# nipponjo/tts-arabic-pytorch

Hardware: AMD Instinct MI355X
Metric: audio samples/sec (FastPitch+HiFi-GAN, synthetic 64-phoneme inputs) (higher is better)
Workload: dtype f32

## Files before the change

tts-arabic-pytorch_amd/csrc/api.hip:

```cpp
#include <cerrno>
#include <cstdio>
#include <cstdlib>
#include <cstring>
#include <algorithm>
#include <atomic>
#include <mutex>
#include <string>
#include <vector>

#include "kernels.hpp"

namespace ttsamd {

static thread_local std::string g_err;

void set_error(const char* fmt, ...) {
    char buf[1024];
    va_list ap;
    va_start(ap, fmt);
    vsnprintf(buf, sizeof(buf), fmt, ap);
    va_end(ap);
    g_err = buf;
}

// ... 436 lines not shown
    TTS_REQUIRE(mode >= 0 && mode <= 2 && (mode != 2 || div != 0.f), "conv1d: bad mode / div");
    TTS_REQUIRE(relu_out == 0 || mode == 0, "conv1d: relu_out with an accumulate mode (mode %d) is not defined", mode);
    hipStream_t s = (hipStream_t)stream;
    const int cp = cout_padded(cout);
    const int64_t n = (int64_t)cin * k * cp;
    hipLaunchKernelGGL(pack_conv_weight_kernel, dim3((unsigned)((n + 255) / 256)), dim3(256), 0, s, w, cout, cin, k,
                       cp, packed);
    TTS_CHECK_HIP(hipGetLastError());
    ConvParams p;
    std::memset(&p, 0, sizeof(p));
    p.x = x; p.x_bs = (int64_t)cin * lin; p.x_cs = lin;
    p.w = packed; p.bias = bias;
    p.precision = default_precision();
    if (p.precision != 0) {
        unsigned short* planes = reinterpret_cast<unsigned short*>(packed + n);
        hipLaunchKernelGGL(split_bf16_kernel, dim3((unsigned)((n + 255) / 256)), dim3(256), 0, s, packed, n, planes);
        TTS_CHECK_HIP(hipGetLastError());
        p.w_bf16 = planes;
    }
    if ((k == 3 || k == 7 || k == 11) && p.precision == 0 && cin % 8 == 0) {
        float* wino = packed + 2 * n;
        const int64_t nw = (int64_t)cin * wino2_groups(k) * cp;
        hipLaunchKernelGGL(pack_wino2_weight_kernel, dim3((unsigned)((nw + 255) / 256)), dim3(256), 0, s, w, cout, cin, k, cp, wino);
        TTS_CHECK_HIP(hipGetLastError());
        p.w_wino = wino;
        float* wino4 = wino + nw;
        const int64_t nw4 = (int64_t)cin * wino4_groups(k) * cp;
        hipLaunchKernelGGL(pack_wino4_weight_kernel, dim3((unsigned)((nw4 + 255) / 256)), dim3(256), 0, s, w, cout, cin, k, cp, wino4);
        TTS_CHECK_HIP(hipGetLastError());
        p.w_wino4 = wino4;
    }
    p.y = y; p.y_bs = (int64_t)cout * lin; p.y_cs = lin; p.y_ts = 1;
    p.lens_in = lens; p.lens_out = lens; p.len_in_mul = 1; p.len_out_mul = 1;
    p.Lin = lin; p.Nout = lin; p.Cin = cin; p.Cout = cout; p.CoutP = cp; p.K = k;
    p.dil = dilation; p.pad = (k * dilation - dilation) / 2;
    p.res = res; p.r_bs = (int64_t)cout * lin; p.r_cs = lin;
    p.n_phase = 1; p.in_slope = in_slope; p.relu_out = relu_out; p.mode = mode; p.div = div; p.batch = batch;
    prof_begin(s, 2.0 * cout * cin * k);
    const int32_t rc = launch_conv(p, s);
    prof_end(s);
    return rc;
}

int32_t ttsamd_conv1d(const float* x, const float* w, const float* bias, const int64_t* lens, int32_t batch,
                      int32_t cin, int32_t cout, int32_t k, int32_t dilation, int32_t lin, float in_slope,
                      int32_t relu_out, float* y, float* packed, void* stream) {
    return ttsamd_conv1d_ex(x, w, bias, nullptr, lens, batch, cin, cout, k, dilation, lin, in_slope, relu_out, 0, 1.f, y, packed, stream);
}

int64_t ttsamd_resblock_pair_packed_floats(int32_t channels, int32_t k, int32_t variant) {
    if (channels < 1 || k < 1) return 0;
    const int64_t n = 2 * (int64_t)channels * k * channels;
    const int nwino = (variant == 4 ? 1 : (variant == 5 ? 2 : 0));
    return n + ((k == 3 || k == 7 || k == 11) ? nwino * (int64_t)channels * wino2_groups(k) * channels : 0);
}

int32_t ttsamd_resblock_pair(const float* x, float* y, const float* w1, const float* b1, const float* w2, const float* b2,
                             int32_t channels, int32_t k, int32_t dil, const int64_t* lens, int32_t len_mul, int32_t L,
                             int32_t batch, int32_t mode, float div, float slope, int32_t variant, float* packed, int64_t packed_floats,
                             void* stream) {
    TTS_REQUIRE(x && y && w1 && b1 && w2 && b2 && packed && channels % 32 == 0 && k >= 1 && batch >= 1 && L >= 1 && len_mul >= 1 &&
                mode >= 0 && mode <= 2, "resblock_pair: bad argument");
    TTS_REQUIRE(packed_floats >= ttsamd_resblock_pair_packed_floats(channels, k, variant),
                "resblock_pair: `packed` holds %lld floats, variant %d at C = %d, k = %d needs %lld (ttsamd_resblock_pair_packed_floats)",
                (long long)packed_floats, variant, channels, k, (long long)ttsamd_resblock_pair_packed_floats(channels, k, variant));
    hipStream_t s = (hipStream_t)stream;
    const int64_t n = (int64_t)channels * k * channels;
    for (int i = 0; i < 2; ++i) {
        hipLaunchKernelGGL(pack_conv_weight_kernel, dim3((unsigned)((n + 255) / 256)), dim3(256), 0, s, i == 0 ? w1 : w2, channels,
                           channels, k, channels, packed + i * n);
        TTS_CHECK_HIP(hipGetLastError());
    }
    const double fl = 2.0 * (2.0 * channels * channels * k);
    int32_t rc;
    prof_begin(s, fl);
    if (variant == 1) {
        rc = launch_fused_pair(channels, x, y, packed, b1, packed + n, b2, k, dil, lens, len_mul, L, batch, mode, div, slope, s);
    } else if (variant >= 2 && variant <= 5) {
        const float *w2w = nullptr, *w1w = nullptr;
        if (variant >= 4) {
            TTS_REQUIRE((k == 3 || k == 7 || k == 11) && (channels <= 64 || (variant == 5 && channels == 128)),
                        "resblock_pair: variants 4 / 5 are built for C = 32 / 64 (5: and 128), k = 3 / 7 / 11");
            const int64_t nw = (int64_t)channels * wino2_groups(k) * channels;
            for (int i = 0; i < (variant == 5 ? 2 : 1); ++i) {
                float* wino = packed + 2 * n + i * nw;
                hipLaunchKernelGGL(pack_wino2_weight_kernel, dim3((unsigned)((nw + 255) / 256)), dim3(256), 0, s, i == 0 ? w2 : w1, channels,
                                   channels, k, channels, wino);
                TTS_CHECK_HIP(hipGetLastError());
                (i == 0 ? w2w : w1w) = wino;
            }
        }
        rc = launch_fused_pair2(channels, x, y, packed, b1, packed + n, b2, k, dil, lens, len_mul, L, batch, mode, div, slope,
                                variant == 3 ? 1 : 2, s, w2w, w1w);
    } else if (variant == -1) {
        rc = 0;
    } else {
        set_error("resblock_pair: variant %d (1: first generation, 2 / 3: second generation with 256- / 128-column blocks, 4 / 5: 256 columns + Winograd phase B / both phases)", variant);
        rc = TTSAMD_EINVAL;
    }
    prof_end(s);
    return rc;
}

int32_t ttsamd_set_precision(int32_t precision) {
    TTS_REQUIRE(precision >= 0 && precision <= 2, "set_precision: 0 = fp32 MFMA, 1 = bf16 MFMA, 2 = split-bf16 MFMA");
    g_precision = precision;
    return 0;
}
int32_t ttsamd_get_precision(void) { return g_precision; }

int32_t ttsamd_profile_enable(int32_t on) {
    std::lock_guard<std::mutex> lk(g_prof.mu);
    g_prof.on = on != 0;
    g_prof.used = 0;
    g_prof.launches = 0;
    g_prof.flops_per_frame = 0.0;
    return 0;
}

int32_t ttsamd_profile_read(double* out3) {
    TTS_REQUIRE(out3, "profile_read: null argument");
    std::lock_guard<std::mutex> lk(g_prof.mu);
    std::vector<std::pair<float, float>> iv;
    for (size_t i = 0; i + 1 < g_prof.used; i += 2) {
        TTS_CHECK_HIP(hipEventSynchronize(g_prof.ev[i + 1]));
        float t0 = 0.f, t1 = 0.f;
        if (i > 0) TTS_CHECK_HIP(hipEventElapsedTime(&t0, g_prof.ev[0], g_prof.ev[i]));
        TTS_CHECK_HIP(hipEventElapsedTime(&t1, g_prof.ev[0], g_prof.ev[i + 1]));
        iv.emplace_back(t0, std::max(t0, t1));
    }
    std::sort(iv.begin(), iv.end());
    double ms = 0.0;
    float lo = 0.f, hi = -1.f;
    for (const auto& v : iv) {
        if (hi < lo || v.first > hi) {
            if (hi >= lo) ms += hi - lo;
            lo = v.first;
            hi = v.second;
        } else {
            hi = std::max(hi, v.second);
        }
    }
    if (hi >= lo) ms += hi - lo;
    out3[0] = ms;
    out3[1] = (double)g_prof.launches;
    out3[2] = (double)(g_prof.used / 2);
    return 0;
}

}
// ... 1 lines not shown
```

tts-arabic-pytorch_amd/csrc/common.hpp:

```cpp
#pragma once
#include <hip/hip_runtime.h>
#include <stdint.h>
#include <atomic>
#include <cstdarg>
#include <cstdio>
#include <cstdlib>
#include <string>

#include "../../include/ttsamd.h"

namespace ttsamd {

void set_error(const char* fmt, ...);

#define TTS_CHECK_HIP(expr)                                                         \
    do {                                                                            \
        hipError_t e_ = (expr);                                                     \
        if (e_ != hipSuccess) {                                                     \
            ttsamd::set_error("%s failed: %s (%s:%d)", #expr, hipGetErrorString(e_), \
                              __FILE__, __LINE__);                                  \
            return TTSAMD_EHIP;                                                     \
        }                                                                           \
    } while (0)

#define TTS_REQUIRE(cond, ...)              \
    do {                                    \
        if (!(cond)) {                      \
            ttsamd::set_error(__VA_ARGS__); \
            return TTSAMD_EINVAL;           \
        }                                   \
    } while (0)

#define TTS_TRY(expr)               \
    do {                            \
        int32_t rc_ = (expr);       \
        if (rc_ != 0) return rc_;   \
    } while (0)

inline int64_t align_up(int64_t x, int64_t a) { return (x + a - 1) / a * a; }

inline const char* exp_env(const char* name) {
#ifdef TTS_EXPERIMENT
    return std::getenv(name);
#else
    (void)name;
    return nullptr;
#endif
}

inline hipError_t lds_opt_in(const void* fn, int bytes, std::atomic<uint64_t>& done) {
    int dev = 0;
    hipError_t e = hipGetDevice(&dev);
    if (e != hipSuccess) return e;
    if (dev >= 0 && dev < 64 && ((done.load(std::memory_order_acquire) >> dev) & 1)) return hipSuccess;
    e = hipFuncSetAttribute(fn, hipFuncAttributeMaxDynamicSharedMemorySize, bytes);
    if (e == hipSuccess && dev >= 0 && dev < 64) done.fetch_or(1ull << dev, std::memory_order_release);
    return e;
}

#define TTS_OPTIONS(X)                                                                                     \
    X(HIFIGAN_STREAMS, 0, 0, 1)    \
    X(WINO, 0, 0, 1)                                              \
    X(WINO2, 0, 0, 31)             \
    X(WINO4, 0, 0, 31)             \
    X(FUSED_PAIR, 0, 0, 1)                   \
    X(FUSED2, 0, 0, 1)                                           \
    X(FUSED2_MASK, 1, 0, 0x1ff)               \
    X(FUSED2_MASK_N1, 1, 0, 0x1ff)          \
    X(FUSED2_WB, 0, 0, 2)                     \
    X(CONVT, 0, 0, 1)                              \
    X(BFO, 0, 0, 1)                \
    X(BFO_CHAIN, 0, 0, 1)                           \
    X(BFO_CHAIN7, 0, 0, 1)                                 \
    X(BFO_FF, 0, 0, 1)                              \
    X(BFO_SPLITK, 0, 0, 1)                                              \
    X(BFO_SMALL_TILES, 0, 0, 1)            \
    X(BF16_ATTN, 0, 0, 1)                                         \
    X(BF16_PACKED_T, 0, 0, 1)                   \
    X(ATT_RA, 0, 1, 4)                             \
    X(ATT_SPLIT, 0, 0, 1)                      \
    X(XCD_W, 0, 0, 1)                            \
    X(XCD_WMAX_KB, 0, 0, 1 << 20)     \
    X(DEEP_SPLITK, 0, 0, 1)        \
    X(TACO_PERSISTENT, 0, 0, 2)    \
    X(TACO_SEG, 0, 8, 1 << 20)
enum Opt : int {
#define TTS_OPT_ENUM(name, kind, lo, hi) OPT_##name,
    TTS_OPTIONS(TTS_OPT_ENUM)
#undef TTS_OPT_ENUM
    OPT_COUNT
};
const char* opt_str(Opt o);

struct Arena {
    char* base;
    int64_t size;
    int64_t off = 0;
    bool ok = true;
    Arena(void* p, int64_t n) : base((char*)p), size(n) {}
    template <typename T>
    T* take(int64_t count) {
        int64_t bytes = align_up(count * (int64_t)sizeof(T), 256);
        if (base != nullptr && off + bytes > size) ok = false;
        T* r = base ? (T*)(base + off) : nullptr;
        off += bytes;
        return r;
    }
};

struct ConvParams {
    const float* x;
    int64_t x_bs;
    int32_t x_cs;
    const float* w;
    const void* w_bf16;
    const float* w_wino;
    const float* w_wino4;
    int32_t precision;
    const float* bias;
    float* y;
    int64_t y_bs;
    int32_t y_cs, y_ts;
    const float* res;
    int64_t r_bs;
    int32_t r_cs;
    const int64_t* lens_in;
    const int64_t* lens_out;
    int32_t len_in_mul, len_out_mul;
    int32_t Lin, Nout;
    int32_t Cin, Cout, CoutP, K;
    int32_t dil, pad;
    int32_t n_phase;
    int32_t phase_p;
    float in_slope;
    const float* scale;
    int32_t relu_out;
    int32_t mode;
    float div;
    int32_t batch;
    float* splitk_ws;
    int64_t splitk_floats;
    int32_t ksplit;
    int32_t y_packed;
    float pack_slope;
    int32_t x_packed;
    int32_t xcd_w;
    int32_t tile_major;
    int32_t compact;
    unsigned long long* timing;
};
constexpr int64_t kSplitKFloats = 4 << 20;
constexpr int64_t kSplitKFloatsFp = 8 << 20;

void conv_log(const char* kind, int K, int cin, int cout, int nout, int batch, int has_res, int mode, int len_mul, int ragged,
              int n_phase);
bool tile_major_order(const ConvParams& p, unsigned n_tiles);
bool compact_order(const void* lens, int batch);
int32_t launch_conv(const ConvParams& p, hipStream_t stream);
bool convt_supported(const ConvParams& p);
int32_t launch_convt(const ConvParams& p, hipStream_t stream);
bool fused_pair_supported(int32_t channels, int32_t k, int32_t dil, int32_t L, const float* x, const float* y);
int32_t launch_fused_pair(int32_t channels, const float* x, float* y, const float* w1, const float* b1, const float* w2,
                          const float* b2, int32_t k, int32_t dil, const int64_t* lens, int32_t len_mul, int32_t L, int32_t batch,
                          int32_t mode, float div, float slope, hipStream_t stream);
bool fused_pair2_supported(int32_t channels, int32_t k, int32_t dil, int32_t L, const float* x, const float* y, int32_t ntw);
int32_t launch_fused_pair2(int32_t channels, const float* x, float* y, const float* w1, const float* b1, const float* w2,
                           const float* b2, int32_t k, int32_t dil, const int64_t* lens, int32_t len_mul, int32_t L, int32_t batch,
                           int32_t mode, float div, float slope, int32_t ntw, hipStream_t stream, const float* w2_wino = nullptr,
                           const float* w1_wino = nullptr);
int wino_route(const ConvParams& p);
int32_t launch_wino(const ConvParams& p, hipStream_t stream);
void pack_wino_weight(const float* w, int cout, int cin, float* out);
int wino2_groups(int k);
int wino2_block_outputs(int coutp, int dil);
int32_t launch_wino2(const ConvParams& p, hipStream_t stream);
void pack_wino2_weight(const float* w, int cout, int cin, int k, float* out);
int wino4_groups(int k);
int wino4_block_outputs(int dil);
int wino4_ksplit(const ConvParams& p);
int32_t launch_splitk_reduce(const ConvParams& q, hipStream_t stream);
int32_t launch_wino4(const ConvParams& p, hipStream_t stream);
void wino4_filter_groups(const float* g, int k, float* o);
void pack_wino4_weight(const float* w, int cout, int cin, int k, float* out);
void pack_conv_weight(const float* w, int cout, int cin, int k, float* out);
void pack_convt_weight(const float* w, int cin, int cout, int kt, int u, int p, float* out);
inline int cout_padded(int cout) { return (int)align_up(cout, 32); }
void split_packed_bf16(const float* packed, int64_t n, uint16_t* out);
int32_t default_precision();

#ifdef __HIPCC__
__device__ __forceinline__ bool live_tile(const int64_t* __restrict__ lens, const int mul, const int n_max, const int tile_w,
                                          const int batch, const unsigned lin, int& b, int& tile) {
    const int lane = threadIdx.x & 63;
    unsigned base = 0;
    for (int u0 = 0; u0 < batch; u0 += 64) {
        int n = 0;
        if (u0 + lane < batch) n = (max(min(n_max, (int)lens[u0 + lane] * mul), 0) + tile_w - 1) / tile_w;
        int incl = n;
#pragma unroll
        for (int d = 1; d < 64; d <<= 1) {
            const int t = __shfl_up(incl, d, 64);
            if (lane >= d) incl += t;
        }
        const unsigned total = (unsigned)__shfl(incl, 63, 64);
        if (lin < base + total) {
            const unsigned long long m = __ballot(base + (unsigned)incl > lin);
            const int l = __ffsll((long long)m) - 1;
            b = u0 + l;
            tile = (int)(lin - base) - (__shfl(incl, l, 64) - __shfl(n, l, 64));
            return true;
        }
        base += total;
    }
    return false;
}
#endif

}
```

tts-arabic-pytorch_amd/csrc/hifigan.hip:

```cpp
#include <cmath>
#include <cstring>
#include <cstdlib>
#include <map>
#include <mutex>
#include <string>
#include <vector>

#include "kernels.hpp"
#include "bfo3.hpp"

namespace ttsamd {

constexpr unsigned kFused2Mask = 0x00F;
constexpr unsigned kFused2MaskN1 = 0x000;
constexpr int64_t kFused2SmallColumns = 2 * 256 * 252;

struct ConvW {
    int64_t w_off = 0, b_off = 0;
    int64_t w16_off = 0, w_n = 0;
    int64_t wo_off = -1;
    int64_t wo3_off = -1;
    int64_t ww4_off = -1;
    int64_t ww_off = -1;
    int cin = 0, cout = 0, k = 0;
};

struct HifiGan {
    ttsamd_hifigan_cfg cfg;
    float* dev = nullptr;
    uint16_t* dev16 = nullptr;
    int64_t dev_n = 0, dev16_n = 0;
    ConvW conv_pre, conv_post;
    std::vector<ConvW> ups;
    std::vector<ConvW> c1, c2;
    int hop = 1;
    int64_t max_cl = 0;
    bool bfo_ok = false;
    mutable std::mutex mu;
    mutable hipStream_t side[2] = {nullptr, nullptr};
    mutable hipEvent_t ev_fork = nullptr, ev_done[3] = {nullptr, nullptr, nullptr};
};

static bool use_branch_streams(const HifiGan* h, int32_t B, int32_t T) {
    if (h->cfg.n_kernels != 3) return false;
    const char* env = opt_str(OPT_HIFIGAN_STREAMS);
    if (env) return env[0] == '1';
    if (default_precision() == 1 && h->bfo_ok) {
        const char* bfo_env = opt_str(OPT_BFO);
        if (!(bfo_env && bfo_env[0] == '0')) return (int64_t)B * T >= 8192;
    }
    return true;
}

struct Fused2Switches {
    bool on = true, mask_forced = false, small_on = false;
    bool wino_b = true, wino_a = true;
    unsigned mask = kFused2Mask, mask_n1 = kFused2MaskN1;
};
static bool parse_hex_mask(const char* txt, unsigned& out) {
    if (!txt || !*txt) return false;
    char* end = nullptr;
    const unsigned long v = std::strtoul(txt, &end, 16);
    if (end == txt || *end != '\0' || v > 0x1ff) return false;
    out = (unsigned)v;
    return true;
}
static int32_t read_fused2_switches(Fused2Switches& sw) {
    const char* e = opt_str(OPT_FUSED2);
    sw.on = !(e && e[0] == '0');
    if (const char* m = opt_str(OPT_FUSED2_MASK)) {
        TTS_REQUIRE(parse_hex_mask(m, sw.mask), "TTSAMD_FUSED2_MASK='%s' is not a hex mask of 9 bits (bit 3 * ci + ki; 1ff = every pair)", m);
        sw.mask_forced = true;
    }
    if (const char* m = opt_str(OPT_FUSED2_MASK_N1))
        TTS_REQUIRE(parse_hex_mask(m, sw.mask_n1), "TTSAMD_FUSED2_MASK_N1='%s' is not a hex mask of 9 bits", m);
    const char* wb = opt_str(OPT_FUSED2_WB);
    sw.wino_b = !(wb && wb[0] == '0');
    sw.wino_a = sw.wino_b && !(wb && wb[0] == '1');
    const char* se = exp_env("TTSAMD_FUSED2_SMALL");
    sw.small_on = se && se[0] == '1';
    return 0;
}

static int fused2_choice(const Fused2Switches& sw, int32_t channels, int32_t k, int32_t dil, int32_t L, const float* x, const float* y,
                         int64_t columns) {
    if (!sw.on) return 0;
    const int ci = channels == 32 ? 0 : (channels == 64 ? 1 : (channels == 128 ? 2 : -1));
    const int ki = k == 3 ? 0 : (k == 7 ? 1 : (k == 11 ? 2 : -1));
    if (ci < 0 || ki < 0) return 0;
    unsigned mask = sw.mask, mask_n1 = sw.mask_n1;
    const unsigned bit = 1u << (3 * ci + ki);
    const bool small = columns < (int64_t)kFused2SmallColumns && !sw.mask_forced;
    if (small) {
        if (!sw.small_on) return 0;
        mask = 0x1ff; mask_n1 = 0x1ff;
    }
    if (!(mask & bit)) return 0;
    int ntw = (mask_n1 & bit) ? 1 : 2;
    if (!fused_pair2_supported(channels, k, dil, L, x, y, ntw)) {
        ntw = 3 - ntw;
        if (!fused_pair2_supported(channels, k, dil, L, x, y, ntw)) return 0;
    }
    return ntw;
}

using TensorMap = std::map<std::string, const ttsamd_tensor*>;

static int64_t numel(const ttsamd_tensor* t) {
    int64_t n = 1;
    for (int i = 0; i < t->ndim; ++i) n *= t->shape[i];
    return n;
}

static int32_t folded_weight(const TensorMap& tm, const std::string& base, int ndim_expected,
                             std::vector<float>& out, int64_t shape[3]) {
    const ttsamd_tensor *w = nullptr, *g = nullptr, *v = nullptr;
    auto it = tm.find(base + ".weight");
    if (it != tm.end()) w = it->second;
    if (!w) {
        auto ig = tm.find(base + ".parametrizations.weight.original0");
        auto iv = tm.find(base + ".parametrizations.weight.original1");
        if (ig == tm.end() || iv == tm.end()) {
            ig = tm.find(base + ".weight_g");
            iv = tm.find(base + ".weight_v");
        }
        TTS_REQUIRE(ig != tm.end() && iv != tm.end(), "hifigan: no weight for layer '%s'", base.c_str());
        g = ig->second;
        v = iv->second;
    }
    const ttsamd_tensor* src = w ? w : v;
    TTS_REQUIRE(src->ndim == ndim_expected, "hifigan: '%s' has ndim %d, expected %d", base.c_str(), src->ndim,
// ... 2 lines not shown
    const int64_t n = numel(src);
    out.resize(n);
    if (w) {
        std::memcpy(out.data(), w->data, n * sizeof(float));
        return 0;
    }
    const int64_t d0 = v->shape[0], inner = n / d0;
    TTS_REQUIRE(numel(g) == d0, "hifigan: '%s' weight_g has %lld elements, expected %lld", base.c_str(),
                (long long)numel(g), (long long)d0);
    for (int64_t i = 0; i < d0; ++i) {
        double ss = 0.0;
        const float* vr = v->data + i * inner;
        for (int64_t j = 0; j < inner; ++j) ss += (double)vr[j] * vr[j];
        const float scale = g->data[i] / (float)std::sqrt(ss);
        for (int64_t j = 0; j < inner; ++j) out[i * inner + j] = vr[j] * scale;
    }
    return 0;
}

static int32_t get_bias(const TensorMap& tm, const std::string& base, int n, std::vector<float>& blob,
                        int64_t& off) {
    auto it = tm.find(base + ".bias");
    TTS_REQUIRE(it != tm.end() && numel(it->second) == n, "hifigan: missing/mis-sized '%s.bias'", base.c_str());
    off = (int64_t)blob.size();
    blob.insert(blob.end(), it->second->data, it->second->data + n);
    blob.resize(align_up((int64_t)blob.size(), 64));
    return 0;
}

static void add_bf16(std::vector<float>& blob, std::vector<uint16_t>& blob16, ConvW& cw, int64_t n) {
    cw.w_n = n;
    cw.w16_off = (int64_t)blob16.size();
    blob16.resize(blob16.size() + 2 * n);
    split_packed_bf16(blob.data() + cw.w_off, n, blob16.data() + cw.w16_off);
}

static int32_t add_conv(const TensorMap& tm, const std::string& base, int cin, int cout, int k,
                        std::vector<float>& blob, std::vector<uint16_t>& blob16, ConvW& cw) {
    std::vector<float> w;
    int64_t shp[3];
    TTS_TRY(folded_weight(tm, base, 3, w, shp));
    TTS_REQUIRE(shp[0] == cout && shp[1] == cin && shp[2] == k, "hifigan: '%s' has shape [%lld,%lld,%lld], expected [%d,%d,%d]",
                base.c_str(), (long long)shp[0], (long long)shp[1], (long long)shp[2], cout, cin, k);
    cw.cin = cin; cw.cout = cout; cw.k = k;
    cw.w_off = (int64_t)blob.size();
    blob.resize(blob.size() + (size_t)cin * k * cout_padded(cout));
    pack_conv_weight(w.data(), cout, cin, k, blob.data() + cw.w_off);
    add_bf16(blob, blob16, cw, (int64_t)cin * k * cout_padded(cout));
    if ((k == 3 || k == 7 || k == 11) && cin % 8 == 0 && cout % 32 == 0) {
        blob.resize(align_up((int64_t)blob.size(), 64));
        cw.ww_off = (int64_t)blob.size();
        blob.resize(blob.size() + (size_t)cin * wino2_groups(k) * cout_padded(cout));
        pack_wino2_weight(w.data(), cout, cin, k, blob.data() + cw.ww_off);
        if (cout >= 64) {
            blob.resize(align_up((int64_t)blob.size(), 64));
            cw.ww4_off = (int64_t)blob.size();
            blob.resize(blob.size() + (size_t)cin * wino4_groups(k) * cout_padded(cout));
            pack_wino4_weight(w.data(), cout, cin, k, blob.data() + cw.ww4_off);
        }
    }
    if (cin % 8 == 0 && cout % 32 == 0) {
        blob16.resize(align_up((int64_t)blob16.size(), 64));
        cw.wo_off = (int64_t)blob16.size();
        blob16.resize(blob16.size() + (size_t)bfo_packed_conv_elems(cout, cin, k));
        bfo_pack_conv_weight(w.data(), cout, cin, k, blob16.data() + cw.wo_off);
        blob16.resize(align_up((int64_t)blob16.size(), 64));
        cw.wo3_off = (int64_t)blob16.size();
        blob16.resize(blob16.size() + (size_t)bfo3_packed_conv_elems(cout, cin, k));
        bfo3_pack_conv_weight(w.data(), cout, cin, k, blob16.data() + cw.wo3_off);
    }
    blob.resize(align_up((int64_t)blob.size(), 64));
    return get_bias(tm, base, cout, blob, cw.b_off);
}

void hifigan_destroy(HifiGan* h);

__global__ void hifigan_touch_kernel() {}

int32_t hifigan_create(const ttsamd_tensor* weights, int32_t n, const ttsamd_hifigan_cfg* cfg, HifiGan** out) {
    TTS_REQUIRE(weights && cfg && out, "hifigan_create: null argument");
    TTS_REQUIRE(cfg->n_ups >= 1 && cfg->n_ups <= 8 && cfg->n_kernels >= 1 && cfg->n_kernels <= 8 &&
                cfg->n_dilations >= 1 && cfg->n_dilations <= 8, "hifigan_create: bad config counts");
    TensorMap tm;
    for (int i = 0; i < n; ++i) tm[weights[i].name] = &weights[i];
    auto* h = new HifiGan();
    h->cfg = *cfg;
    std::vector<float> blob;
    std::vector<uint16_t> blob16;
    const int c0 = cfg->upsample_initial_channel;
    int32_t rc = add_conv(tm, "conv_pre", cfg->num_mels, c0, 7, blob, blob16, h->conv_pre);
    int ch = c0, mul = 1;
    h->max_cl = c0;
    for (int i = 0; rc == 0 && i < cfg->n_ups; ++i) {
        const int u = cfg->upsample_rates[i], kt = cfg->upsample_kernel_sizes[i];
        const int cin = ch, cout = ch / 2;
        if (kt != 2 * u || (kt - u) % 2 != 0) {
            set_error("hifigan: upsample kernel %d / rate %d: only kernel = 2*rate is built", kt, u);
            rc = TTSAMD_EINVAL;
            break;
        }
        std::vector<float> w;
        int64_t shp[3];
        rc = folded_weight(tm, "ups." + std::to_string(i), 3, w, shp);
        if (rc) break;
        if (shp[0] != cin || shp[1] != cout || shp[2] != kt) {
            set_error("hifigan: ups.%d has shape [%lld,%lld,%lld], expected [%d,%d,%d]", i, (long long)shp[0],
                      (long long)shp[1], (long long)shp[2], cin, cout, kt);
// ... 133 lines not shown
    const int nb = multi ? 3 : 1;
    float* cur = a.take<float>((int64_t)B * h->max_cl * T);
    float* ups_out = a.take<float>((int64_t)B * h->max_cl * T);
    float *Tbs[3], *Rs[3], *splitks[3];
    for (int i = 0; i < nb; ++i) {
        Tbs[i] = a.take<float>((int64_t)B * h->max_cl * T);
        Rs[i] = a.take<float>((int64_t)B * h->max_cl * T);
    }
    for (int i = 0; i < nb; ++i) splitks[i] = a.take<float>(kSplitKFloats);
    for (int i = nb; i < 3; ++i) { Tbs[i] = Tbs[0]; Rs[i] = Rs[0]; splitks[i] = splitks[0]; }
    uint16_t* mel_o = a.take<uint16_t>((int64_t)B * align_up(h->cfg.num_mels, 8) * T * 2);
    if (!ws || !a.ok) {
        set_error("hifigan_forward: workspace of %lld bytes needed, %lld given", (long long)a.off, (long long)ws_bytes);
        return TTSAMD_ENOMEM;
    }
    const ttsamd_hifigan_cfg& cfg = h->cfg;
    std::unique_lock<std::mutex> lk(h->mu, std::defer_lock);
    hipStream_t bs[3] = {s, s, s};
    if (multi) {
        lk.lock();
        TTS_REQUIRE(h->ev_fork && h->side[0] && h->side[1], "hifigan_forward: the branch streams were not created (hifigan_create)");
        bs[1] = h->side[0];
        bs[2] = h->side[1];
    }

    struct Join {
        bool on; hipStream_t a, b;
        ~Join() { if (on) { (void)hipStreamSynchronize(a); (void)hipStreamSynchronize(b); } }
    } join{false, bs[1], bs[2]};
    const auto fail = [&](int32_t rc) { join.on = multi && rc != 0; return rc; };

    ConvParams p;
    std::memset(&p, 0, sizeof(p));
    p.batch = B;
    p.lens_in = lens; p.lens_out = lens;
    p.n_phase = 1; p.div = 1.f;
    p.splitk_ws = splitks[0]; p.splitk_floats = kSplitKFloats;
    const char* pk_env = opt_str(OPT_BF16_PACKED_T);
    const bool pack_t = default_precision() == 1 && !(pk_env && pk_env[0] == '0');
    Fused2Switches f2sw;
    TTS_TRY(read_fused2_switches(f2sw));
    const char* fz_env = opt_str(OPT_FUSED_PAIR);
    const bool fused_ok = default_precision() == 0 && !(fz_env && fz_env[0] == '0');
    const char* ct_env = opt_str(OPT_CONVT);
    const bool convt_ok = !(ct_env && ct_env[0] == '0');
    bool in_section = false;
    int pack_io = 0;
    auto conv = [&](const ConvW& cw, const float* x, hipStream_t st, float* y, const float* res, int L, int mul,
                    int dil, float slope, int mode, float div) -> int32_t {
        p.x = x; p.x_bs = (int64_t)cw.cin * L; p.x_cs = L;
        p.w = h->dev + cw.w_off; p.bias = h->dev + cw.b_off;
        p.w_bf16 = h->dev16 + cw.w16_off; p.precision = default_precision();
        p.w_wino = cw.ww_off >= 0 ? h->dev + cw.ww_off : nullptr;
        p.w_wino4 = cw.ww4_off >= 0 ? h->dev + cw.ww4_off : nullptr;
        p.y = y; p.y_bs = (int64_t)cw.cout * L; p.y_cs = L; p.y_ts = 1;
        p.res = res; p.r_bs = (int64_t)cw.cout * L; p.r_cs = L;
        p.len_in_mul = mul; p.len_out_mul = mul; p.Lin = L; p.Nout = L;
        p.Cin = cw.cin; p.Cout = cw.cout; p.CoutP = cout_padded(cw.cout); p.K = cw.k;
        p.dil = dil; p.pad = (cw.k * dil - dil) / 2;
        p.n_phase = 1; p.phase_p = 0;
        p.in_slope = slope; p.relu_out = 0; p.mode = mode; p.div = div;
        p.x_packed = (pack_io & 1) ? 1 : 0; p.y_packed = (pack_io & 2) ? 1 : 0; p.pack_slope = 0.1f;
        if (in_section) prof_add(2.0 * cw.cout * cw.cin * cw.k * mul);
        else prof_begin(st, 2.0 * cw.cout * cw.cin * cw.k * mul);
        const int32_t rc = launch_conv(p, st);
        if (!in_section) prof_end(st);
        return rc;
    };

#define HG_TRY(expr) do { int32_t rc_ = (expr); if (rc_ != 0) return fail(rc_); } while (0)
#define HG_CHECK_HIP(expr) do { hipError_t e_ = (expr); if (e_ != hipSuccess) { set_error("%s failed: %s (%s:%d)", #expr, hipGetErrorString(e_), __FILE__, __LINE__); return fail(TTSAMD_EHIP); } } while (0)
    const char* bfo_env = opt_str(OPT_BFO);
    const int prec = default_precision();
    if ((prec == 1 || prec == 2) && h->bfo_ok && !(bfo_env && bfo_env[0] == '0')) {
        const bool x3 = prec == 2;
        const uint16_t* W16 = h->dev16;
        const auto woff = [x3](const ConvW& cw) { return x3 ? cw.wo3_off : cw.wo_off; };
        const auto l_conv = x3 ? bfo3_launch_conv : bfo_launch_conv;
        const auto l_convt = x3 ? bfo3_launch_convt : bfo_launch_convt;
        const auto l_pair = x3 ? bfo3_launch_pair : bfo_launch_pair;
        const auto pair_ok = x3 ? bfo3_pair_supported : bfo_pair_supported;
        const char* c3e = opt_str(OPT_BFO_CHAIN);
        const bool chain3_on = !(c3e && c3e[0] == '0');
        void *curo = cur, *upso = ups_out;
        HG_TRY((x3 ? bfo3_launch_pack : bfo_launch_pack)(mel, B, cfg.num_mels, T, 1.f, mel_o, s));
        BfoConvParams cp;
        std::memset(&cp, 0, sizeof(cp));
        cp.batch = B; cp.lens = lens; cp.div = 1.f; cp.res_slope = 1.f;
        cp.x = mel_o; cp.y = curo; cp.w = W16 + woff(h->conv_pre); cp.bias = h->dev + h->conv_pre.b_off;
        cp.len_mul = 1; cp.Lin = T; cp.Cin = h->conv_pre.cin; cp.Cout = h->conv_pre.cout; cp.K = 7; cp.dil = 1; cp.up = 1;
        cp.mode = 0; cp.out_slope = 0.1f;
        prof_begin(s, 2.0 * cp.Cout * cp.Cin * 7);
        int32_t rc = l_conv(cp, s);
        prof_end(s);
        HG_TRY(rc);
        int L = T, mul = 1;
        for (int i = 0; i < cfg.n_ups; ++i) {
            const int u = cfg.upsample_rates[i];
            const ConvW& uw = h->ups[i];
            cp.x = curo; cp.y = upso; cp.w = W16 + woff(uw); cp.bias = h->dev + uw.b_off; cp.res = nullptr; cp.sum_in = nullptr;
            cp.len_mul = mul; cp.Lin = L; cp.Cin = uw.cin; cp.Cout = uw.cout; cp.K = 2; cp.dil = 1; cp.up = u;
            cp.mode = 0; cp.out_slope = 0.1f;
            prof_begin(s, 2.0 * uw.cout * uw.cin * 2 * u * mul);
            rc = l_convt(cp, s);
            prof_end(s);
            HG_TRY(rc);
            L *= u; mul *= u;
// ... 79 lines not shown
                }
            }
            if (multi) {
                HG_CHECK_HIP(hipStreamWaitEvent(s, h->ev_done[cfg.n_kernels - 1], 0));
                in_section = false;
                prof_section_end(s);
            }
        }
        HG_TRY((x3 ? bfo3_launch_conv_post : bfo_launch_conv_post)(curo, h->dev + h->conv_post.w_off, h->dev + h->conv_post.b_off, lens, mul, B, h->conv_post.cin,
                                    L, wave, (int64_t)L, s));
        return 0;
    }

    HG_TRY(conv(h->conv_pre, mel, s, cur, nullptr, T, 1, 1, 1.0f, 0, 1.f));
    int L = T, mul = 1;
    for (int i = 0; i < cfg.n_ups; ++i) {
        const int u = cfg.upsample_rates[i], kt = cfg.upsample_kernel_sizes[i];
        const ConvW& uw = h->ups[i];
        p.x = cur; p.x_bs = (int64_t)uw.cin * L; p.x_cs = L;
        p.w = h->dev + uw.w_off; p.bias = h->dev + uw.b_off;
        p.w_bf16 = h->dev16 + uw.w16_off; p.precision = default_precision(); p.w_wino = nullptr; p.w_wino4 = nullptr;
        p.y = ups_out; p.y_bs = (int64_t)uw.cout * L * u; p.y_cs = L * u; p.y_ts = u;
        p.res = nullptr;
        p.len_in_mul = mul; p.len_out_mul = mul; p.Lin = L; p.Nout = L;
        p.Cin = uw.cin; p.Cout = uw.cout; p.CoutP = cout_padded(uw.cout); p.K = 2;
        p.dil = -1; p.pad = 0; p.n_phase = u; p.phase_p = (kt - u) / 2;
        p.in_slope = 0.1f; p.relu_out = 0; p.mode = 0; p.div = 1.f;
        p.x_packed = 0; p.y_packed = 0;
        prof_begin(s, 2.0 * uw.cout * uw.cin * 2 * u * mul);
        int32_t rc = (convt_ok && convt_supported(p)) ? launch_convt(p, s) : launch_conv(p, s);
        prof_end(s);
        HG_TRY(rc);
        L *= u; mul *= u;
        if (multi) {
            prof_section_begin(s);
            in_section = true;
            HG_CHECK_HIP(hipEventRecord(h->ev_fork, s));
        }
        for (int j = 0; j < cfg.n_kernels; ++j) {
            hipStream_t st = bs[j % 3];
            float *Tb = Tbs[j % 3], *R = Rs[j % 3];
            p.splitk_ws = splitks[j % 3];
            if (multi && j > 0) HG_CHECK_HIP(hipStreamWaitEvent(st, h->ev_fork, 0));
            const float* src = ups_out;
            for (int m = 0; m < cfg.n_dilations; ++m) {
                const int li = (i * cfg.n_kernels + j) * cfg.n_dilations + m;
                const int d = cfg.resblock_dilations[j][m];
                {
                    const bool last = m + 1 == cfg.n_dilations;
                    float* dst = last ? cur : (src == R ? Tb : R);
                    const ConvW &w1 = h->c1[li], &w2 = h->c2[li];
                    const bool square = w1.cin == w1.cout && w2.cin == w1.cin && w2.cout == w1.cin && w1.k == w2.k;
                    const int ntw2 = (fused_ok && square) ? fused2_choice(f2sw, w1.cin, w1.k, d, L, src, dst, (int64_t)B * L) : 0;
                    if (ntw2 != 0 || (fused_ok && square && fused_pair_supported(w1.cin, w1.k, d, L, src, dst))) {
                        const int mode = !last ? 0 : (cfg.n_kernels == 1 ? 0 : (j == 0 ? 0 : (j + 1 < cfg.n_kernels ? 1 : 2)));
                        if (multi && last && j > 0) HG_CHECK_HIP(hipStreamWaitEvent(st, h->ev_done[j - 1], 0));
                        const double fl = 2.0 * (2.0 * w1.cin * w1.cin * w1.k) * mul;
                        if (in_section) prof_add(fl); else prof_begin(st, fl);
                        const int32_t frc = ntw2 != 0
                            ? launch_fused_pair2(w1.cin, src, dst, h->dev + w1.w_off, h->dev + w1.b_off, h->dev + w2.w_off,
                                                 h->dev + w2.b_off, w1.k, d, lens, mul, L, B, mode, (float)cfg.n_kernels, 0.1f, ntw2, st,
                                                 (f2sw.wino_b && w2.ww_off >= 0) ? h->dev + w2.ww_off : nullptr,
                                                 (f2sw.wino_a && w1.ww_off >= 0) ? h->dev + w1.ww_off : nullptr)
                            : launch_fused_pair(w1.cin, src, dst, h->dev + w1.w_off, h->dev + w1.b_off, h->dev + w2.w_off,
                                                h->dev + w2.b_off, w1.k, d, lens, mul, L, B, mode, (float)cfg.n_kernels, 0.1f, st);
                        if (!in_section) prof_end(st);
                        HG_TRY(frc);
                        if (multi && last) HG_CHECK_HIP(hipEventRecord(h->ev_done[j], st));
                        src = dst;
                        continue;
                    }
                }
                pack_io = pack_t ? 2 : 0;
                HG_TRY(conv(h->c1[li], src, st, Tb, nullptr, L, mul, d, 0.1f, 0, 1.f));
                pack_io = pack_t ? 1 : 0;
                if (m + 1 < cfg.n_dilations) {
                    HG_TRY(conv(h->c2[li], Tb, st, R, src, L, mul, 1, 0.1f, 0, 1.f));
                    pack_io = 0;
                    src = R;
                } else {
                    const int mode = (j == 0) ? 0 : (j + 1 < cfg.n_kernels ? 1 : 2);
                    const int md = cfg.n_kernels == 1 ? 0 : mode;
                    if (multi && j > 0) HG_CHECK_HIP(hipStreamWaitEvent(st, h->ev_done[j - 1], 0));
                    HG_TRY(conv(h->c2[li], Tb, st, cur, src, L, mul, 1, 0.1f, md, (float)cfg.n_kernels));
                    pack_io = 0;
                    if (multi) HG_CHECK_HIP(hipEventRecord(h->ev_done[j], st));
                }
            }
        }
        p.splitk_ws = splitks[0];
        if (multi) {
            HG_CHECK_HIP(hipStreamWaitEvent(s, h->ev_done[cfg.n_kernels - 1], 0));
            in_section = false;
            prof_section_end(s);
        }
    }
    HG_TRY(launch_conv_post(cur, (int64_t)h->conv_post.cin * L, L, h->dev + h->conv_post.w_off,
                             h->dev + h->conv_post.b_off, lens, mul, B, h->conv_post.cin, L, 0.01f, wave,
                             (int64_t)L, s));
#undef HG_TRY
#undef HG_CHECK_HIP
    return 0;
}

void hifigan_blobs(const void* hv, void** f32, int64_t* n_f32, void** b16, int64_t* n_b16) {
    const HifiGan* h = (const HifiGan*)hv;
    *f32 = h->dev; *n_f32 = h->dev_n; *b16 = h->dev16; *n_b16 = h->dev16_n;
}

}
```

Before: 69.65 million.

## Add Winograd F(4,3) fused ResBlock pair kernel for 32-channel HiFi-GAN stages

Adds a new fused ResBlock-pair kernel for C=32 that runs both convolutions through Winograd F(4,3) transforms on fp32 MFMA, with LDS-staged activations and a prefetched weight queue. It is routed by default for k>=7 when the 256-column second-generation path is selected and Winograd is enabled. It also packs F(4,3) weights for those layers and keeps the generic conv path from picking them up. The aim is to cut the MFMA work of the final low-channel, long-sequence resblocks. The cost is extra weight memory, more transform arithmetic, and F(4,3) numerical error in fp32.

```diff
diff --git a/tts-arabic-pytorch_amd/csrc/api.hip b/tts-arabic-pytorch_amd/csrc/api.hip
--- a/tts-arabic-pytorch_amd/csrc/api.hip
+++ b/tts-arabic-pytorch_amd/csrc/api.hip
@@ -512,6 +512,7 @@
     if (channels < 1 || k < 1) return 0;
     const int64_t n = 2 * (int64_t)channels * k * channels;
     const int nwino = (variant == 4 ? 1 : (variant == 5 ? 2 : 0));
+    if (variant == 6) return n + ((k == 3 || k == 7 || k == 11) ? 2 * (int64_t)channels * wino4_groups(k) * channels : 0);
     return n + ((k == 3 || k == 7 || k == 11) ? nwino * (int64_t)channels * wino2_groups(k) * channels : 0);
 }
 
@@ -552,10 +553,20 @@
         }
         rc = launch_fused_pair2(channels, x, y, packed, b1, packed + n, b2, k, dil, lens, len_mul, L, batch, mode, div, slope,
                                 variant == 3 ? 1 : 2, s, w2w, w1w);
+    } else if (variant == 6) {
+        TTS_REQUIRE(channels == 32 && (k == 3 || k == 7 || k == 11), "resblock_pair: variant 6 is built for C = 32, k = 3 / 7 / 11");
+        const int64_t nw4 = (int64_t)channels * wino4_groups(k) * channels;
+        for (int i = 0; i < 2; ++i) {
+            hipLaunchKernelGGL(pack_wino4_weight_kernel, dim3((unsigned)((nw4 + 255) / 256)), dim3(256), 0, s, i == 0 ? w1 : w2, channels,
+                               channels, k, channels, packed + 2 * n + i * nw4);
+            TTS_CHECK_HIP(hipGetLastError());
+        }
+        rc = launch_fused_pair4(channels, x, y, packed + 2 * n, b1, packed + 2 * n + nw4, b2, k, dil, lens, len_mul, L, batch, mode, div,
+                                slope, s);
     } else if (variant == -1) {
         rc = 0;
     } else {
-        set_error("resblock_pair: variant %d (1: first generation, 2 / 3: second generation with 256- / 128-column blocks, 4 / 5: 256 columns + Winograd phase B / both phases)", variant);
+        set_error("resblock_pair: variant %d (1: first generation, 2 / 3: second generation with 256- / 128-column blocks, 4 / 5: 256 columns + Winograd phase B / both phases, 6: C = 32 with both phases on Winograd F(4,3))", variant);
         rc = TTSAMD_EINVAL;
     }
     prof_end(s);
diff --git a/tts-arabic-pytorch_amd/csrc/common.hpp b/tts-arabic-pytorch_amd/csrc/common.hpp
--- a/tts-arabic-pytorch_amd/csrc/common.hpp
+++ b/tts-arabic-pytorch_amd/csrc/common.hpp
@@ -68,6 +68,7 @@
     X(FUSED2_MASK, 1, 0, 0x1ff)               \
     X(FUSED2_MASK_N1, 1, 0, 0x1ff)          \
     X(FUSED2_WB, 0, 0, 2)                     \
+    X(PAIR4, 0, 0, 1)              \
     X(CONVT, 0, 0, 1)                              \
     X(BFO, 0, 0, 1)                \
     X(BFO_CHAIN, 0, 0, 1)                           \
@@ -168,6 +169,10 @@
                            const float* b2, int32_t k, int32_t dil, const int64_t* lens, int32_t len_mul, int32_t L, int32_t batch,
                            int32_t mode, float div, float slope, int32_t ntw, hipStream_t stream, const float* w2_wino = nullptr,
                            const float* w1_wino = nullptr);
+bool fused_pair4_supported(int32_t channels, int32_t k, int32_t dil, int32_t L, const float* x, const float* y);
+int32_t launch_fused_pair4(int32_t channels, const float* x, float* y, const float* w1_wino4, const float* b1, const float* w2_wino4,
+                           const float* b2, int32_t k, int32_t dil, const int64_t* lens, int32_t len_mul, int32_t L, int32_t batch,
+                           int32_t mode, float div, float slope, hipStream_t stream);
 int wino_route(const ConvParams& p);
 int32_t launch_wino(const ConvParams& p, hipStream_t stream);
 void pack_wino_weight(const float* w, int cout, int cin, float* out);
diff --git a/tts-arabic-pytorch_amd/csrc/hifigan.hip b/tts-arabic-pytorch_amd/csrc/hifigan.hip
--- a/tts-arabic-pytorch_amd/csrc/hifigan.hip
+++ b/tts-arabic-pytorch_amd/csrc/hifigan.hip
@@ -12,6 +12,7 @@
 namespace ttsamd {
 
 constexpr unsigned kFused2Mask = 0x00F;
+constexpr int kPair4MinK = 7;
 constexpr unsigned kFused2MaskN1 = 0x000;
 constexpr int64_t kFused2SmallColumns = 2 * 256 * 252;
 
@@ -55,6 +56,7 @@
 struct Fused2Switches {
     bool on = true, mask_forced = false, small_on = false;
     bool wino_b = true, wino_a = true;
+    bool pair4 = true;
     unsigned mask = kFused2Mask, mask_n1 = kFused2MaskN1;
 };
 static bool parse_hex_mask(const char* txt, unsigned& out) {
@@ -77,6 +79,8 @@
     const char* wb = opt_str(OPT_FUSED2_WB);
     sw.wino_b = !(wb && wb[0] == '0');
     sw.wino_a = sw.wino_b && !(wb && wb[0] == '1');
+    const char* p4 = opt_str(OPT_PAIR4);
+    sw.pair4 = !(p4 && p4[0] == '0');
     const char* se = exp_env("TTSAMD_FUSED2_SMALL");
     sw.small_on = se && se[0] == '1';
     return 0;
@@ -185,7 +189,7 @@
         cw.ww_off = (int64_t)blob.size();
         blob.resize(blob.size() + (size_t)cin * wino2_groups(k) * cout_padded(cout));
         pack_wino2_weight(w.data(), cout, cin, k, blob.data() + cw.ww_off);
-        if (cout >= 64) {
+        if (cout >= 64 || (cout == 32 && cin == 32 && k >= kPair4MinK)) {
             blob.resize(align_up((int64_t)blob.size(), 64));
             cw.ww4_off = (int64_t)blob.size();
             blob.resize(blob.size() + (size_t)cin * wino4_groups(k) * cout_padded(cout));
@@ -425,7 +429,7 @@
         p.w = h->dev + cw.w_off; p.bias = h->dev + cw.b_off;
         p.w_bf16 = h->dev16 + cw.w16_off; p.precision = default_precision();
         p.w_wino = cw.ww_off >= 0 ? h->dev + cw.ww_off : nullptr;
-        p.w_wino4 = cw.ww4_off >= 0 ? h->dev + cw.ww4_off : nullptr;
+        p.w_wino4 = (cw.ww4_off >= 0 && cw.cout >= 64) ? h->dev + cw.ww4_off : nullptr;
         p.y = y; p.y_bs = (int64_t)cw.cout * L; p.y_cs = L; p.y_ts = 1;
         p.res = res; p.r_bs = (int64_t)cw.cout * L; p.r_cs = L;
         p.len_in_mul = mul; p.len_out_mul = mul; p.Lin = L; p.Nout = L;
@@ -611,12 +615,17 @@
                     const ConvW &w1 = h->c1[li], &w2 = h->c2[li];
                     const bool square = w1.cin == w1.cout && w2.cin == w1.cin && w2.cout == w1.cin && w1.k == w2.k;
                     const int ntw2 = (fused_ok && square) ? fused2_choice(f2sw, w1.cin, w1.k, d, L, src, dst, (int64_t)B * L) : 0;
+                    const bool f43 = ntw2 == 2 && f2sw.pair4 && f2sw.wino_a && w1.k >= kPair4MinK && w1.ww4_off >= 0 && w2.ww4_off >= 0 &&
+                                     fused_pair4_supported(w1.cin, w1.k, d, L, src, dst);
                     if (ntw2 != 0 || (fused_ok && square && fused_pair_supported(w1.cin, w1.k, d, L, src, dst))) {
                         const int mode = !last ? 0 : (cfg.n_kernels == 1 ? 0 : (j == 0 ? 0 : (j + 1 < cfg.n_kernels ? 1 : 2)));
                         if (multi && last && j > 0) HG_CHECK_HIP(hipStreamWaitEvent(st, h->ev_done[j - 1], 0));
                         const double fl = 2.0 * (2.0 * w1.cin * w1.cin * w1.k) * mul;
                         if (in_section) prof_add(fl); else prof_begin(st, fl);
-                        const int32_t frc = ntw2 != 0
+                        const int32_t frc = f43
+                            ? launch_fused_pair4(w1.cin, src, dst, h->dev + w1.ww4_off, h->dev + w1.b_off, h->dev + w2.ww4_off,
+                                                 h->dev + w2.b_off, w1.k, d, lens, mul, L, B, mode, (float)cfg.n_kernels, 0.1f, st)
+                            : ntw2 != 0
                             ? launch_fused_pair2(w1.cin, src, dst, h->dev + w1.w_off, h->dev + w1.b_off, h->dev + w2.w_off,
                                                  h->dev + w2.b_off, w1.k, d, lens, mul, L, B, mode, (float)cfg.n_kernels, 0.1f, ntw2, st,
                                                  (f2sw.wino_b && w2.ww_off >= 0) ? h->dev + w2.ww_off : nullptr,
diff --git a/tts-arabic-pytorch_amd/csrc/resblock_pair4.hip b/tts-arabic-pytorch_amd/csrc/resblock_pair4.hip
--- /dev/null
+++ b/tts-arabic-pytorch_amd/csrc/resblock_pair4.hip
@@ -0,0 +1,343 @@
+#include <algorithm>
+#include <cstring>
+
+#include "conv_mfma_common.hpp"
+#include "bfo.hpp"
+
+namespace ttsamd {
+
+struct FusedPair4Params {
+    const float* x;
+    float* y;
+    const float4* w1;
+    const float4* w2;
+    const float* b1;
+    const float* b2;
+    const int64_t* lens;
+    int32_t len_mul, L, dil, batch;
+    int32_t mode;
+    float div, slope;
+    int32_t compact;
+};
+
+template <int K>
+struct Pair4Geo {
+    static constexpr int C = 32, NOCT = C / 8;
+    static constexpr int H = (K - 1) / 2;
+    static constexpr int NSF = K == 3 ? 1 : (K == 7 ? 2 : 4);
+    static constexpr int NTAP = K == 7 ? 4 : 0;
+    static constexpr int NG = K == 3 ? 6 : (K == 7 ? 16 : 23);
+    static constexpr int NGQ = (NG + 1) & ~1;
+    static constexpr int NPL = K == 7 ? 8 : 6;
+    static constexpr int NPOS = K + 3;
+    static constexpr int NBU = NSF + (NTAP ? 1 : 0);
+    static constexpr int PF = 4;
+    static constexpr int UO = (NGQ % PF == 0) ? 1 : 2;
+    static_assert((UO * NGQ) % PF == 0 && NOCT % UO == 0, "queue slots");
+    static constexpr int NQ = 128;
+    static constexpr int WQ = 145;
+    static constexpr int ROW = 4 * WQ;
+    static constexpr int LDS_BYTES = 2 * NOCT * ROW * 16;
+    static_assert(LDS_BYTES <= 80 * 1024, "two blocks per CU");
+    __host__ __device__ static constexpr int nqa(int d) { return (4 * NQ / (4 * d)) * d; }
+    __host__ __device__ static constexpr int ts(int d) { return (4 * nqa(d) - 2 * H) & ~3; }
+    __host__ __device__ static constexpr int nvec(int d) { return (3 + 4 * nqa(d) + (K - 1) * d + 3) / 4; }
+    static_assert(nvec(1) <= WQ && nvec(3) <= WQ && nvec(5) <= WQ, "window fits a sub-row");
+    static_assert((4 * NQ - 4 + NPOS - 1) / 4 < WQ, "phase B reads stay inside a sub-row");
+    __host__ __device__ static constexpr int bpos(int u) { return u < NSF ? 3 * u : 3 * NSF; }
+    __host__ __device__ static constexpr int bnum(int u) { return u < NSF ? (3 * u + 5 < NPOS ? 6 : 5) : 4; }
+};
+
+__device__ __forceinline__ float p4_lrelu(const float v, const float slope) {
+    return __builtin_amdgcn_fmed3f(v, v * slope, __builtin_inff());
+}
+
+typedef float p4_f4 __attribute__((ext_vector_type(4)));
+
+__device__ __forceinline__ p4_f4 p4v(const float4 a) { return p4_f4{a.x, a.y, a.z, a.w}; }
+
+template <int K>
+__device__ __forceinline__ void p4_conv(f32x16 (&acc)[Pair4Geo<K>::NPL], float4 (&aq)[Pair4Geo<K>::PF], const float4* xs,
+                                        const int (&eo)[Pair4Geo<K>::NPOS], const float4* __restrict__ wl,
+                                        const float4* __restrict__ wnext) {
+    using G = Pair4Geo<K>;
+    constexpr int C = G::C, NOCT = G::NOCT, NSF = G::NSF, NGQ = G::NGQ, PF = G::PF, UO = G::UO, NBU = G::NBU, ROW = G::ROW;
+    constexpr int NGT = NOCT * NGQ;
+    float4 xq[2][6];
+#pragma unroll
+    for (int m = 0; m < G::bnum(0); ++m) xq[0][m] = xs[eo[G::bpos(0) + m]];
+#pragma unroll 1
+    for (int ob = 0; ob < NOCT; ob += UO) {
+#pragma unroll
+        for (int bi = 0; bi < UO * NBU; ++bi) {
+            const int ol = bi / NBU, u = bi % NBU, cur = bi & 1, nxt = cur ^ 1;
+            const int o = ob + ol;
+            {
+                const int un = (u + 1) % NBU;
+                const int on = min(u + 1 < NBU ? o : o + 1, NOCT - 1);
+                const float4* xn = xs + on * 2 * ROW;
+#pragma unroll
+                for (int m = 0; m < G::bnum(un); ++m) xq[nxt][m] = xn[eo[G::bpos(un) + m]];
+            }
+            p4_f4 x[6];
+#pragma unroll
+            for (int m = 0; m < G::bnum(u); ++m) x[m] = p4v(xq[cur][m]);
+            const bool sub = u < NSF;
+            const int ng = sub ? 6 : 4;
+#pragma unroll
+            for (int i = 0; i < ng; ++i) {
+                const int g = sub ? 6 * u + i : 6 * NSF + i;
+                const int gb = ol * NGQ + g;
+                const int slot = gb % PF;
+                const float4 a4 = aq[slot];
+                {
+                    const int gn = o * NGQ + g + PF;
+                    const float4* __restrict__ src = gn < NGT ? wl + gn * 2 * C : wnext + (gn - NGT) * 2 * C;
+                    aq[slot] = *src;
+                }
+                if (g >= G::NG) continue;
+                p4_f4 v;
+                int plane;
+                if (sub) {
+                    plane = i;
+                    if (i == 0) v = 4.f * x[0] + (x[4] - 5.f * x[2]);
+                    else if (i == 1) v = (x[4] - 4.f * x[2]) + (x[3] - 4.f * x[1]);
+                    else if (i == 2) v = (x[4] - 4.f * x[2]) - (x[3] - 4.f * x[1]);
+                    else if (i == 3) v = (x[4] - x[2]) + 2.f * (x[3] - x[1]);
+                    else if (i == 4) v = (x[4] - x[2]) - 2.f * (x[3] - x[1]);
+                    else v = 4.f * x[1] + (x[5] - 5.f * x[3]);
+                } else {
+                    plane = i == 0 ? 0 : (i == 1 ? 6 : (i == 2 ? 7 : 5));
+                    v = x[i];
+                }
+                __builtin_amdgcn_sched_barrier(0);
+                const float av[4] = {a4.x, a4.y, a4.z, a4.w};
+#pragma unroll
+                for (int pq = 0; pq < 4; ++pq) acc[plane] = __builtin_amdgcn_mfma_f32_32x32x2f32(av[pq], v[pq], acc[plane], 0, 0, 0);
+            }
+        }
+        if ((UO * NBU) & 1) {
+#pragma unroll
+            for (int m = 0; m < 6; ++m) xq[0][m] = xq[1][m];
+        }
+    }
+}
+
+template <int NPL>
+__device__ __forceinline__ void p4_out(const f32x16 (&acc)[NPL], const int r, float (&y)[4]) {
+    const float s12 = acc[1][r] + acc[2][r], d12 = acc[1][r] - acc[2][r];
+    const float s34 = acc[3][r] + acc[4][r], d34 = acc[3][r] - acc[4][r];
+    y[0] = acc[0][r] + s12 + s34;
+    y[1] = d12 + 2.f * d34;
+    y[2] = s12 + 4.f * s34;
+    y[3] = d12 + 8.f * d34 + acc[5][r];
+    if constexpr (NPL == 8) {
+        y[1] += acc[6][r];
+        y[2] += acc[7][r];
+    }
+}
+
+template <int K>
+__global__ __launch_bounds__(256, 2) void resblock_pair4(const FusedPair4Params p) {
+    using G = Pair4Geo<K>;
+    constexpr int C = G::C, NOCT = G::NOCT, H = G::H, NPL = G::NPL, NPOS = G::NPOS, PF = G::PF, WQ = G::WQ, ROW = G::ROW;
+    extern __shared__ __attribute__((aligned(16))) float4 smem4[];
+    const int dil = p.dil, L = p.L;
+    const int TS = G::ts(dil);
+    const int tid = threadIdx.x, lane = tid & 63, wid = tid >> 6;
+    const int kk = lane >> 5, l31 = lane & 31;
+    int b = blockIdx.z;
+    int q0 = blockIdx.x * TS;
+    if (p.compact) {
+        int tile = 0;
+        if (!live_tile(p.lens, p.len_mul, L, TS, p.batch, blockIdx.z * gridDim.x + blockIdx.x, b, tile)) return;
+        b = __builtin_amdgcn_readfirstlane(b);
+        q0 = __builtin_amdgcn_readfirstlane(tile) * TS;
+    }
+    int len = L;
+    if (p.lens) len = min(len, (int)p.lens[b] * p.len_mul);
+    if (q0 >= len) return;
+    const float slope = p.slope;
+    const float* __restrict__ xb = p.x + (int64_t)b * C * L;
+    float4* Xs = smem4;
+
+    const float4* __restrict__ wl1 = p.w1 + kk * C + l31;
+    const float4* __restrict__ wl2 = p.w2 + kk * C + l31;
+    float4 aq[PF];
+#pragma unroll
+    for (int g = 0; g < PF; ++g) aq[g] = wl1[g * 2 * C];
+
+    const int xfirst = q0 - H - H * dil;
+    const int xa = xfirst & ~3, off = xfirst - xa;
+    {
+        const int nv = G::nvec(dil), n_items = 2 * NOCT * nv;
+        constexpr int NE = (2 * NOCT * G::WQ + 255) / 256;
+        float4 v[NE][4];
+#pragma unroll
+        for (int u = 0; u < NE; ++u) {
+            const int it = tid + 256 * u;
+            const int row = min(it / nv, 2 * NOCT - 1), vi = it - row * nv;
+            const int ch0 = 8 * (row >> 1) + (row & 1);
+            const int voff = it < n_items ? (xa + 4 * vi) * 4 : BFO_OOB;
+#pragma unroll
+            for (int pq = 0; pq < 4; ++pq) {
+                const bfo_i4 rs = bfo_rsrc(xb + (int64_t)(ch0 + 2 * pq) * L, (unsigned)max(len, 0) * 4u);
+                v[u][pq] = __builtin_bit_cast(float4, bfo_ld16(rs, voff, 0, 0));
+            }
+        }
+#pragma unroll
+        for (int u = 0; u < NE; ++u) {
+            const int it = tid + 256 * u;
+            if (it < n_items) {
+                const int row = it / nv, vi = it - row * nv;
+                const float vv[4][4] = {{v[u][0].x, v[u][0].y, v[u][0].z, v[u][0].w}, {v[u][1].x, v[u][1].y, v[u][1].z, v[u][1].w},
+                                        {v[u][2].x, v[u][2].y, v[u][2].z, v[u][2].w}, {v[u][3].x, v[u][3].y, v[u][3].z, v[u][3].w}};
+#pragma unroll
+                for (int j = 0; j < 4; ++j)
+                    Xs[row * ROW + j * WQ + vi] = make_float4(p4_lrelu(vv[0][j], slope), p4_lrelu(vv[1][j], slope),
+                                                              p4_lrelu(vv[2][j], slope), p4_lrelu(vv[3][j], slope));
+            }
+        }
+    }
+    __syncthreads();
+
+    const int jw = wid * 32 + l31;
+    const int nqa = G::nqa(dil);
+    const int pa = min(jw, nqa - 1);
+    const int na = dil == 1 ? 4 * pa : (pa / dil) * 4 * dil + pa % dil;
+    f32x16 acc[NPL];
+#pragma unroll
+    for (int g = 0; g < NPL; ++g)
+#pragma unroll
+        for (int r = 0; r < 16; ++r) acc[g][r] = 0.f;
+    {
+        int eo[NPOS];
+#pragma unroll
+        for (int m = 0; m < NPOS; ++m) {
+            const int c = off + na + m * dil;
+            eo[m] = (c & 3) * WQ + (c >> 2);
+        }
+        p4_conv<K>(acc, aq, Xs + kk * ROW, eo, wl1, wl2);
+    }
+    __syncthreads();
+    if (jw < nqa) {
+        float bias[16];
+#pragma unroll
+        for (int r = 0; r < 16; ++r) bias[r] = p.b1[(r & 3) + 8 * (r >> 2) + 4 * kk];
+        float y[16][4];
+#pragma unroll
+        for (int r = 0; r < 16; ++r) p4_out<NPL>(acc, r, y[r]);
+#pragma unroll
+        for (int h = 0; h < 4; ++h) {
+            const int c = na + h * dil;
+            const int pos = q0 - H + c;
+            const bool live = pos >= 0 && pos < len;
+            const int ent = (c & 3) * WQ + (c >> 2);
+#pragma unroll
+            for (int oc = 0; oc < 4; ++oc)
+#pragma unroll
+                for (int k2 = 0; k2 < 2; ++k2) {
+                    const int r = 4 * oc + k2;
+                    const float v0 = p4_lrelu(y[r][h] + bias[r], slope), v1 = p4_lrelu(y[r + 2][h] + bias[r + 2], slope);
+                    const float2 w2v = live ? make_float2(v0, v1) : make_float2(0.f, 0.f);
+                    *reinterpret_cast<float2*>(reinterpret_cast<float*>(Xs + (2 * oc + k2) * ROW + ent) + 2 * kk) = w2v;
+                }
+        }
+    }
+    __syncthreads();
+
+#pragma unroll
+    for (int g = 0; g < NPL; ++g)
+#pragma unroll
+        for (int r = 0; r < 16; ++r) acc[g][r] = 0.f;
+    {
+        int eo[NPOS];
+#pragma unroll
+        for (int m = 0; m < NPOS; ++m) eo[m] = (m & 3) * WQ + jw + (m >> 2);
+        p4_conv<K>(acc, aq, Xs + kk * ROW, eo, wl2, wl2);
+    }
+
+    const int n = 4 * jw, q = q0 + n;
+    if (n >= TS || q >= len) return;
+    const bool full = q + 3 < len;
+    float* __restrict__ yb = p.y + (int64_t)b * C * L;
+    const int mode = p.mode;
+    const float div = p.div;
+#pragma unroll
+    for (int r = 0; r < 16; ++r) {
+        const int ch = (r & 3) + 8 * (r >> 2) + 4 * kk;
+        float v[4];
+        p4_out<NPL>(acc, r, v);
+        const float bs = p.b2[ch];
+        const float* xp = xb + (int64_t)ch * L + q;
+        float* yp = yb + (int64_t)ch * L + q;
+        float xr[4] = {0.f, 0.f, 0.f, 0.f}, yr[4] = {0.f, 0.f, 0.f, 0.f};
+        if (full) {
+            const float4 t = *reinterpret_cast<const float4*>(xp);
+            xr[0] = t.x; xr[1] = t.y; xr[2] = t.z; xr[3] = t.w;
+            if (mode != 0) { const float4 s = *reinterpret_cast<const float4*>(yp); yr[0] = s.x; yr[1] = s.y; yr[2] = s.z; yr[3] = s.w; }
+        } else {
+#pragma unroll
+            for (int e = 0; e < 4; ++e)
+                if (q + e < len) {
+                    xr[e] = xp[e];
+                    if (mode != 0) yr[e] = yp[e];
+                }
+        }
+#pragma unroll
+        for (int e = 0; e < 4; ++e) {
+            float t = v[e] + bs + xr[e];
+            if (mode == 1) t = yr[e] + t;
+            else if (mode == 2) t = (yr[e] + t) / div;
+            v[e] = t;
+        }
+        if (full) {
+            *reinterpret_cast<float4*>(yp) = make_float4(v[0], v[1], v[2], v[3]);
+        } else {
+#pragma unroll
+            for (int e = 0; e < 4; ++e)
+                if (q + e < len) yp[e] = v[e];
+        }
+    }
+}
+
+template <int K>
+static int32_t launch_pair4_k(const FusedPair4Params& p, hipStream_t stream) {
+    using G = Pair4Geo<K>;
+    static std::atomic<uint64_t> lds_done{0};
+    TTS_CHECK_HIP(lds_opt_in((const void*)resblock_pair4<K>, G::LDS_BYTES, lds_done));
+    const int ts = G::ts(p.dil);
+    dim3 grid((p.L + ts - 1) / ts, 1, p.batch);
+    hipLaunchKernelGGL(resblock_pair4<K>, grid, dim3(256), G::LDS_BYTES, stream, p);
+    TTS_CHECK_HIP(hipGetLastError());
+    return 0;
+}
+
+bool fused_pair4_supported(int32_t channels, int32_t k, int32_t dil, int32_t L, const float* x, const float* y) {
+    if (channels != 32 || !(k == 3 || k == 7 || k == 11) || !(dil == 1 || dil == 3 || dil == 5)) return false;
+    if (L < 4 || (L & 3) != 0 || ((((uintptr_t)x) | ((uintptr_t)y)) & 15) != 0 || x == y) return false;
+    return (int64_t)channels * L * 4 < ((int64_t)1 << 31);
+}
+
+int32_t launch_fused_pair4(int32_t channels, const float* x, float* y, const float* w1_wino4, const float* b1, const float* w2_wino4,
+                           const float* b2, int32_t k, int32_t dil, const int64_t* lens, int32_t len_mul, int32_t L, int32_t batch,
+                           int32_t mode, float div, float slope, hipStream_t stream) {
+    TTS_REQUIRE(fused_pair4_supported(channels, k, dil, L, x, y),
+                "fused ResBlock pair (F(4,3)): unsupported geometry (C=%d, k=%d, dil=%d, L=%d)", channels, k, dil, L);
+    TTS_REQUIRE(w1_wino4 && w2_wino4 && b1 && b2, "fused ResBlock pair (F(4,3)): null weights");
+    TTS_REQUIRE(slope > 0.f && slope <= 1.f, "fused ResBlock pair (F(4,3)): leaky-relu slope %g outside (0, 1]", (double)slope);
+    TTS_REQUIRE(mode >= 0 && mode <= 2 && (mode != 2 || div != 0.f), "fused ResBlock pair (F(4,3)): bad mode / div");
+    conv_log("fused_pair4", k, channels, channels, L, batch, 1, mode, len_mul, lens != nullptr, 1);
+    FusedPair4Params p;
+    std::memset(&p, 0, sizeof(p));
+    p.x = x; p.y = y;
+    p.w1 = reinterpret_cast<const float4*>(w1_wino4); p.w2 = reinterpret_cast<const float4*>(w2_wino4);
+    p.b1 = b1; p.b2 = b2; p.lens = lens; p.len_mul = len_mul; p.L = L; p.dil = dil; p.batch = batch;
+    p.mode = mode; p.div = div; p.slope = slope;
+    p.compact = compact_order(lens, batch) ? 1 : 0;
+    if (k == 3) return launch_pair4_k<3>(p, stream);
+    if (k == 7) return launch_pair4_k<7>(p, stream);
+    return launch_pair4_k<11>(p, stream);
+}
+
+}
```

Result: faster. 71.05 million (median of 6 runs) (+2.0%).
